# consensus-nexus/bayesian-consensus-engine

Measured on AMD Instinct MI355X. Metric: signals aggregated/sec (node) at 1M markets×32 signals; % of HBM roofline, higher is better.
Workload: dtype f64; 1 GPU; c2: 1000000 markets x 32 signals, 10000 sources, batched consensus + validation + sourceWeights outputs, mode=exact; markets_per_gpu=1000000, signals_per_market=32, parallelism=markets sharded, 1 independent rank(s), no collective

## Files before the change

### bayesian-consensus-engine_amd/csrc/consensus_tab.hip

```cpp
#include <stdio.h>
#include <stdlib.h>

#include <algorithm>

#include "consensus_common.hpp"

#pragma clang fp contract(off)

namespace bce {
namespace {

constexpr int kTabWaves = 8;
constexpr bool kTabMetaEarly = true;
constexpr int kPL = 8;
constexpr int kLB = 3;
constexpr int kMG = 64 / kPL;
constexpr int kTabRing = 8;

typedef unsigned tab_u4v __attribute__((ext_vector_type(4)));
typedef double tab_d2v __attribute__((ext_vector_type(2)));
__device__ __forceinline__ uint4 tab_ld16(const uint32_t* p) {
  const tab_u4v v = __builtin_nontemporal_load(reinterpret_cast<const tab_u4v*>(p));
  return make_uint4(v.x, v.y, v.z, v.w);
}
__device__ __forceinline__ void tab_st16(int32_t* p, uint4 v) {
  const tab_u4v x = {v.x, v.y, v.z, v.w};
  __builtin_nontemporal_store(x, reinterpret_cast<tab_u4v*>(p));
}
__device__ __forceinline__ void tab_st16(double* p, double x0, double x1) {
  const tab_d2v x = {x0, x1};
  __builtin_nontemporal_store(x, reinterpret_cast<tab_d2v*>(p));
}

__device__ __forceinline__ void bfly_pl32(uint32_t& a, uint32_t& b) {
  const auto r = __builtin_amdgcn_permlane32_swap(a, b, false, false);
  a = r[0];
  b = r[1];
}
__device__ __forceinline__ void bfly_pl16(uint32_t& a, uint32_t& b) {
  const auto r = __builtin_amdgcn_permlane16_swap(a, b, false, false);
  a = r[0];
  b = r[1];
}
__device__ __forceinline__ void bfly_r8(uint32_t& a, uint32_t& b, int lane) {
  const bool hi = (lane & 8) != 0;
  const uint32_t bx = (uint32_t)__builtin_amdgcn_mov_dpp((int)b, 0x128, 0xF, 0xF, true);
  const uint32_t ax = (uint32_t)__builtin_amdgcn_mov_dpp((int)a, 0x128, 0xF, 0xF, true);
  const uint32_t na = hi ? bx : a;
  b = hi ? b : ax;
  a = na;
}
template <int N>
__device__ __forceinline__ void xpose(uint32_t (&r)[N], int lane) {
#pragma unroll
  for (int i = 0; i < N; ++i)
    if (!(i & 16)) bfly_pl32(r[i], r[i | 16]);
#pragma unroll
  for (int i = 0; i < N; ++i)
    if (!(i & 8)) bfly_pl16(r[i], r[i | 8]);
#pragma unroll
  for (int i = 0; i < N; ++i)
    if (!(i & 4)) bfly_r8(r[i], r[i | 4], lane);
}

__device__ __forceinline__ int tmkt(int lane) { return lane; }
__device__ __forceinline__ int lq(int lane) { return lane & 7; }
__device__ __forceinline__ int lc(int lane) { return lane >> 3; }
__device__ __forceinline__ void oem_sort_kv31(unsigned (&key)[32], double (&val)[32]) {
  constexpr auto P = OemNet<32>::make();
#pragma unroll
  for (int c = 0; c < OemNet<32>::C; ++c) {
    const unsigned x = key[P.a[c]], y = key[P.b[c]];
    unsigned m = (unsigned)((int)(y - x) >> 31);
    asm("" : "+v"(m));
    key[P.a[c]] = min(x, y);
    key[P.b[c]] = max(x, y);
    const uint64_t vx = (uint64_t)__double_as_longlong(val[P.a[c]]), vy = (uint64_t)__double_as_longlong(val[P.b[c]]);
    const uint64_t mm = ((uint64_t)m << 32) | m;
    val[P.a[c]] = __longlong_as_double((long long)((mm & vy) | (~mm & vx)));
    val[P.b[c]] = __longlong_as_double((long long)((mm & vx) | (~mm & vy)));
  }
}

__device__ __forceinline__ double dbl(uint32_t lo, uint32_t hi) {
  return __hiloint2double((int)hi, (int)lo);
}
__device__ __forceinline__ uint32_t lo32(double x) { return (uint32_t)__double_as_longlong(x); }
__device__ __forceinline__ uint32_t hi32(double x) { return (uint32_t)((uint64_t)__double_as_longlong(x) >> 32); }

template <bool HYB>
__global__ __launch_bounds__(64 * kTabWaves) void consensus_tab32_kernel(ConsArgs a) {
  extern __shared__ __attribute__((aligned(16))) unsigned char tab_smem[];
  const int S = a.n_sources > 0 ? a.n_sources : 1;
  const int nwords = (S + 31) >> 5;
  const int rows = HYB ? a.tab_rows : S;
  double2* const sT = reinterpret_cast<double2*>(tab_smem);
  uint32_t* const sB = reinterpret_cast<uint32_t*>(tab_smem + 16 * (size_t)rows);
  if (a.n_sources > 0) {
    int i = threadIdx.x;
    for (; i + 3 * 64 * kTabWaves < rows; i += 4 * 64 * kTabWaves) {
      double2 v[4];
#pragma unroll
      for (int q = 0; q < 4; ++q) v[q] = a.relconf[i + q * 64 * kTabWaves];
#pragma unroll
      for (int q = 0; q < 4; ++q) sT[i + q * 64 * kTabWaves] = v[q];
    }
    for (; i < rows; i += 64 * kTabWaves) sT[i] = a.relconf[i];
    for (int j = threadIdx.x; j < nwords; j += 64 * kTabWaves) sB[j] = a.pbits[j];
  } else if (threadIdx.x == 0) {
    sT[0] = make_double2(0.5, 0.25);
    sB[0] = 0u;
  }
  __syncthreads();

  const int w = __builtin_amdgcn_readfirstlane((int)(threadIdx.x >> 6));
  const unsigned smax = (unsigned)(S - 1);
  const int64_t M = a.n_list;
  const int64_t n_tiles = (M + 63) >> 6;
  const int64_t stride = (int64_t)gridDim.x * kTabWaves;
  const bool do_u = a.usid != nullptr, do_w = a.weight != nullptr, do_nw = a.nweight != nullptr;
  const bool do_any = do_u || do_w || do_nw;

  struct Meta {
    int64_t off;
    int n;
    int64_t B;
    bool reg;
  };
  auto meta = [&](int64_t tile, int lane) -> Meta {
    Meta m{0, 0, 0, false};
    if (tile >= n_tiles) return m;
    const int j = tmkt(lane);
    const int64_t mk = tile * 64 + j;
    int64_t end = 0;
    if (mk < M) {
      m.off = a.offsets[mk];
      end = a.offsets[mk + 1];
    }
    m.n = (int)(end - m.off);
    if (ballot(mk < M && (m.n < 0 || m.n > 32))) {
      raise_fault(a.fault, kFaultTooLong);
      if (m.n < 0 || m.n > 32) m.n = 0;
    }
    m.B = ((int64_t)__builtin_amdgcn_readfirstlane((int)(m.off >> 32)) << 32) |
          (uint32_t)__builtin_amdgcn_readfirstlane((int)m.off);
    m.reg = ballot(!(mk < M && m.n == 32 && m.off == m.B + 32 * (int64_t)j)) == 0 &&
            ((((uintptr_t)(a.sid + m.B)) | ((uintptr_t)(a.prob + m.B))) & 15) == 0;
    return m;
  };
  auto load_regular = [&](int64_t B, int lane, uint32_t (&rs)[32], uint32_t (&rp)[64]) {
    const int q = lq(lane), c = lc(lane);
    const uint32_t* sb = reinterpret_cast<const uint32_t*>(a.sid + B);
    const double* pb = a.prob + B;
#pragma unroll
    for (int k = 0; k < 8; ++k) {
      const uint4 v = tab_ld16(sb + 32 * (kMG * (k & (kPL - 1)) + q) + 4 * kPL * (k >> kLB) + 4 * c);
      rs[4 * k] = v.x; rs[4 * k + 1] = v.y; rs[4 * k + 2] = v.z; rs[4 * k + 3] = v.w;
    }
#pragma unroll
    for (int k = 0; k < 16; ++k) {
      const uint4 v = tab_ld16(reinterpret_cast<const uint32_t*>(pb + 32 * (kMG * (k & (kPL - 1)) + q) +
                                                                 2 * kPL * (k >> kLB) + 2 * c));
      rp[4 * k] = v.x; rp[4 * k + 1] = v.y; rp[4 * k + 2] = v.z; rp[4 * k + 3] = v.w;
    }
  };

  int64_t tile = (int64_t)w * gridDim.x + blockIdx.x;
  Meta cur = meta(tile, lane_id());
  uint32_t s[32], pw[64];
  for (; tile < n_tiles; tile += stride) {
    int lane = lane_id();
    asm volatile("" : "+v"(lane));
    const int64_t m0 = tile * 64;
    const int64_t off = cur.off, B = cur.B;
    const int n = cur.n;
    const bool reg = cur.reg;
    Meta nxt{};
    if constexpr (kTabMetaEarly) nxt = meta(tile + stride, lane);

    if (reg) {
      load_regular(B, lane, s, pw);
      xpose<32>(s, lane);
      xpose<64>(pw, lane);
    } else if (a.n_signals > 0) {
      const int64_t base = (n > 0) ? off : 0;
      const int last = (n > 0) ? n - 1 : 0;
#pragma unroll
      for (int t = 0; t < 32; ++t) {
        const int64_t i = base + min(t, last);
        s[t] = (uint32_t)a.sid[i];
        const double v = a.prob[i];
        pw[2 * t] = lo32(v);
        pw[2 * t + 1] = hi32(v);
      }
    } else {
#pragma unroll
      for (int t = 0; t < 64; ++t) pw[t] = 0u;
#pragma unroll
      for (int t = 0; t < 32; ++t) s[t] = 0u;
    }
    __builtin_amdgcn_sched_barrier(0);
    double p[32];
#pragma unroll
    for (int t = 0; t < 32; ++t) p[t] = dbl(pw[2 * t], pw[2 * t + 1]);

    const unsigned vb = (n >= 32) ? 0xFFFFFFFFu : ((1u << n) - 1u);
    unsigned badp = 0, bads = 0;
#pragma unroll
    for (int t = 0; t < 32; ++t) {
      badp |= ((p[t] < 0.0 || p[t] > 1.0) ? 1u : 0u) << t;
      bads |= ((s[t] > smax) ? 1u : 0u) << t;
    }
    badp &= vb;
    const int err = badp ? (int)__builtin_ctz(badp) : -1;
    if (ballot((bads & vb) != 0u)) raise_fault(a.fault, kFaultSid);

    unsigned key[32];
#pragma unroll
    for (int t = 0; t < 32; ++t) {
      const uint32_t m = (uint32_t)__builtin_amdgcn_sbfe(vb, t, 1);
      key[t] = (m & ((min(s[t], smax) << 5) | (unsigned)t)) | (~m & 0x7FFFFFFFu);
    }
    oem_sort_kv31(key, p);
    __builtin_amdgcn_sched_barrier(0);
    unsigned nq = 0;
#pragma unroll
    for (int t = 30; t >= 0; --t) nq = (nq << 1) | ((((key[t] ^ key[t + 1]) >> 5) != 0u) ? 1u : 0u);
    const unsigned lb = (nq | 0x80000000u) & vb;
    const unsigned fb = ((nq << 1) | 1u) & vb;

    unsigned dupend = lb & ~fb;
    while (ballot(dupend != 0u)) {
      const int te = dupend ? 31 - __builtin_clz(dupend) : -1;
      const unsigned upto = (te >= 0) ? (0xFFFFFFFFu >> (31 - te)) : 0u;
      dupend &= ~(upto ^ (upto >> 1));
      const unsigned fm = fb & upto;
      const int ts = fm ? 31 - __builtin_clz(fm) : 0;
      const unsigned run = upto & ~((1u << ts) - 1u);
      double psum = 0.0;
#pragma unroll
      for (int t = 0; t < 32; ++t) {
        uint32_t m = (uint32_t)__builtin_amdgcn_sbfe(run, t, 1);
        asm("" : "+v"(m));
        const uint64_t m64 = ((uint64_t)m << 32) | m;
        psum += __longlong_as_double((long long)(m64 & (uint64_t)__double_as_longlong(p[t])));
      }
      const double avg = psum / (double)(te - ts + 1);
      const unsigned at = upto ^ (upto >> 1);
#pragma unroll
      for (int t = 0; t < 32; ++t) {
        uint32_t m = (uint32_t)__builtin_amdgcn_sbfe(at, t, 1);
        asm("" : "+v"(m));
        const uint64_t m64 = ((uint64_t)m << 32) | m;
        p[t] = __longlong_as_double((long long)((m64 & (uint64_t)__double_as_longlong(avg)) |
                                                (~m64 & (uint64_t)__double_as_longlong(p[t]))));
      }
    }
    __builtin_amdgcn_sched_barrier(0);

    __builtin_amdgcn_s_setprio(1);
    double2 ring[kTabRing];
    uint32_t rbits[kTabRing];
    auto row = [&](unsigned ix) -> double2 {
      if constexpr (HYB) {
        if (ix >= (unsigned)rows) return a.relconf[ix];
      }
      return sT[ix];
    };
#pragma unroll
    for (int t = 0; t < kTabRing; ++t) {
      const unsigned ix = min(key[t] >> 5, smax);
      ring[t] = row(ix);
      rbits[t] = sB[ix >> 5];
    }
    double total = 0.0, ws = 0.0, cs = 0.0;
#pragma unroll
    for (int t = 0; t < 32; ++t) {
      const unsigned sid = key[t] >> 5;
      const double2 rc = ring[t % kTabRing];
      const uint32_t bw = rbits[t % kTabRing];
      if (t + kTabRing < 32) {
        const unsigned ix = min(key[t + kTabRing < 32 ? t + kTabRing : t] >> 5, smax);
        ring[t % kTabRing] = row(ix);
        rbits[t % kTabRing] = sB[ix >> 5];
      }
      const double wt = rc.x, cf = rc.y, avg = p[t];
      const bool lst = ((lb >> t) & 1u) != 0u;
      total += lst ? wt : 0.0;
      ws += lst ? avg * wt : 0.0;
      cs += lst ? cf * wt : 0.0;
      key[t] = sid | ((((bw >> (sid & 31)) & 1u) != 0u) ? 0u : 0x80000000u);
      p[t] = wt;
      asm volatile("" : "+v"(total), "+v"(ws), "+v"(cs));
      __builtin_amdgcn_sched_barrier(0);
    }
    const int u = __builtin_popcount(lb);

    __builtin_amdgcn_s_setprio(2);
    if constexpr (!kTabMetaEarly) nxt = meta(tile + stride, lane_id());
    {
      int ln = lane_id();
      asm volatile("" : "+v"(ln));
      const int64_t mk2 = m0 + tmkt(ln);
      if (mk2 < M) {
        const bool null_ = (total == 0.0);
        a.consensus[mk2] = null_ ? 0.0 : ws / total;
        a.confidence[mk2] = null_ ? 0.0 : cs / total;
        a.total_weight[mk2] = total;
        a.n_unique[mk2] = u;
        if (a.err_idx) a.err_idx[mk2] = err;
      }
    }
    if (!do_any) {
      __builtin_amdgcn_s_setprio(0);
      cur = nxt;
      continue;
    }

    const unsigned full = (u >= 32) ? 0xFFFFFFFFu : ((1u << u) - 1u);
    if (ballot(lb != full)) {
      unsigned holes = vb & ~lb;
      while (ballot(holes != 0u)) {
        const int h = holes ? 31 - __builtin_clz(holes) : 32;
        holes &= ~(1u << (h & 31));
#pragma unroll
        for (int i = 0; i < 31; ++i) {
          uint32_t m = (uint32_t)((h - 1 - i) >> 31);
          asm("" : "+v"(m));
          key[i] = (m & key[i + 1]) | (~m & key[i]);
          const uint64_t m64 = ((uint64_t)m << 32) | m;
          const uint64_t x = (uint64_t)__double_as_longlong(p[i + 1]), y = (uint64_t)__double_as_longlong(p[i]);
          p[i] = __longlong_as_double((long long)((m64 & x) | (~m64 & y)));
        }
      }
    }

    __builtin_amdgcn_s_setprio(3);
    __builtin_amdgcn_sched_barrier(0);
    if (reg) {
      uint32_t blo = (uint32_t)B, bhi = (uint32_t)((uint64_t)B >> 32);
      asm volatile("" : "+s"(blo), "+s"(bhi));
      const int64_t B = (int64_t)(((uint64_t)bhi << 32) | blo);
      int lane = lane_id();
      asm volatile("" : "+v"(lane));
      const int q = lq(lane), c = lc(lane);
      int uk[kPL];
      double tk[kPL];
#pragma unroll
      for (int k = 0; k < kPL; ++k) {
        const int src = ((k << 3) | (lane & 7)) << 2;
        uk[k] = __builtin_amdgcn_ds_bpermute(src, u);
        tk[k] = dbl((uint32_t)__builtin_amdgcn_ds_bpermute(src, (int)lo32(total)),
                    (uint32_t)__builtin_amdgcn_ds_bpermute(src, (int)hi32(total)));
      }
      if (do_u) {
        uint32_t o[32];
#pragma unroll
        for (int t = 0; t < 32; ++t) o[t] = key[t];
        xpose<32>(o, lane);
#pragma unroll
        for (int k = 0; k < 8; ++k) {
          const int slot = 4 * kPL * (k >> kLB) + 4 * c;
          if (uk[k & (kPL - 1)] > slot)
            tab_st16(a.usid + B + 32 * (kMG * (k & (kPL - 1)) + q) + slot,
                     make_uint4(o[4 * k], o[4 * k + 1], o[4 * k + 2], o[4 * k + 3]));
        }
      }
      if (do_w || do_nw) {
        uint32_t o[64];
#pragma unroll
        for (int t = 0; t < 32; ++t) {
          o[2 * t] = lo32(p[t]);
          o[2 * t + 1] = hi32(p[t]);
        }
        xpose<64>(o, lane);
#pragma unroll
        for (int k = 0; k < 16; ++k) {
          const int slot = 2 * kPL * (k >> kLB) + 2 * c;
          const int64_t pos = B + 32 * (kMG * (k & (kPL - 1)) + q) + slot;
          const double w0 = dbl(o[4 * k], o[4 * k + 1]), w1 = dbl(o[4 * k + 2], o[4 * k + 3]);
          const double tot = tk[k & (kPL - 1)];
          if (uk[k & (kPL - 1)] > slot) {
            if (do_w) tab_st16(a.weight + pos, w0, w1);
            if (do_nw) tab_st16(a.nweight + pos, tot > 0.0 ? w0 / tot : 0.0, tot > 0.0 ? w1 / tot : 0.0);
          }
        }
      }
    } else {
      int ln = lane_id();
      asm volatile("" : "+v"(ln));
      const int64_t mk2 = m0 + tmkt(ln);
      const int64_t off = (mk2 < M) ? a.offsets[mk2] : 0;
#pragma unroll
      for (int j = 0; j < 32; ++j) {
        if (j < u) {
          if (do_u) a.usid[off + j] = (int32_t)key[j];
          if (do_w) a.weight[off + j] = p[j];
        }
      }
      if (do_nw) {
#pragma unroll
        for (int j = 0; j < 32; ++j) {
          const double v = total > 0.0 ? p[j] / total : 0.0;
          if (j < u) a.nweight[off + j] = v;
        }
      }
    }
    __builtin_amdgcn_s_setprio(0);
    cur = nxt;
  }
}

}


template <bool HYB>
int launch_tab32_t(ConsArgs a, hipStream_t st) {
  const int64_t tiles = (a.n_list + 63) / 64;
  if (tiles == 0) return BCE_OK;
  const int S = a.n_sources > 0 ? a.n_sources : 1;
  const size_t bits = 4 * (size_t)((S + 31) / 32);
  a.tab_rows = HYB ? (int)std::min<size_t>(((size_t)kTabLdsBytes - bits) / 16, (size_t)S) : S;
  const size_t lds = 16 * (size_t)a.tab_rows + bits;
  const void* fn = reinterpret_cast<const void*>(&consensus_tab32_kernel<HYB>);
  const int rc = ensure_dynamic_lds(fn, kTabLdsBytes);
  if (rc) return rc;
  const int per_cu = blocks_per_cu(fn, 64 * kTabWaves, lds, 1, HYB ? "consensus_tab32_kernel<hybrid>"
                                                                  : "consensus_tab32_kernel");
  const int64_t blocks = (tiles + kTabWaves - 1) / kTabWaves;
  const int64_t cap = (int64_t)cu_count() * per_cu;
  const int grid = (int)(blocks < cap ? blocks : cap);
  hipLaunchKernelGGL((consensus_tab32_kernel<HYB>), dim3(grid), dim3(64 * kTabWaves), lds, st, a);
  return check_launch("consensus_tab32_kernel");
}

int launch_tab32(const ConsArgs& a, hipStream_t st) {
  return (a.n_sources <= kTabMaxSources) ? launch_tab32_t<false>(a, st) : launch_tab32_t<true>(a, st);
}

}
```

Measured before the change: 149.3 billion signals/s.

## Specialize tile body for regular tiles and overlap offsets prefetch with loads

Splits the per-tile loop body into a compile-time specialized lambda for regular (full 32-signal, contiguous) tiles and an irregular fallback. This drops the validity-mask work in key construction for the common case. Offset metadata is now issued as raw loads and finished later. The first tile's offsets load overlaps the LDS table fill, and the next tile's offsets load is issued after the bulk signal loads so it sits behind them. Metadata is kept in scalar registers, but duplicating the body roughly doubles code size and may raise instruction-cache and register pressure.

New measurement: 151.1 billion signals/s, median of 3. About the same (+1.2%).

```diff
diff --git a/bayesian-consensus-engine_amd/csrc/consensus_tab.hip b/bayesian-consensus-engine_amd/csrc/consensus_tab.hip
--- a/bayesian-consensus-engine_amd/csrc/consensus_tab.hip
+++ b/bayesian-consensus-engine_amd/csrc/consensus_tab.hip
@@ -2,6 +2,7 @@
 #include <stdlib.h>
 
 #include <algorithm>
+#include <type_traits>
 
 #include "consensus_common.hpp"
 
@@ -11,7 +12,6 @@
 namespace {
 
 constexpr int kTabWaves = 8;
-constexpr bool kTabMetaEarly = true;
 constexpr int kPL = 8;
 constexpr int kLB = 3;
 constexpr int kMG = 64 / kPL;
@@ -82,6 +82,12 @@
   }
 }
 
+__device__ __forceinline__ int lane_here() {
+  unsigned ones = ~0u;
+  asm volatile("" : "+s"(ones));
+  return (int)__builtin_amdgcn_mbcnt_hi(ones, __builtin_amdgcn_mbcnt_lo(ones, 0u));
+}
+
 __device__ __forceinline__ double dbl(uint32_t lo, uint32_t hi) {
   return __hiloint2double((int)hi, (int)lo);
 }
@@ -96,6 +102,18 @@
   const int rows = HYB ? a.tab_rows : S;
   double2* const sT = reinterpret_cast<double2*>(tab_smem);
   uint32_t* const sB = reinterpret_cast<uint32_t*>(tab_smem + 16 * (size_t)rows);
+  const int w = __builtin_amdgcn_readfirstlane((int)(threadIdx.x >> 6));
+  const int64_t M = a.n_list;
+  const int64_t n_tiles = (M + 63) >> 6;
+  int64_t tile = (int64_t)w * gridDim.x + blockIdx.x;
+  struct RawMeta {
+    int64_t off, end;
+  };
+  auto meta_issue = [&](int64_t t, int lane) -> RawMeta {
+    const int64_t mk = min(t * 64 + tmkt(lane), M - 1);
+    return RawMeta{a.offsets[mk], a.offsets[mk + 1]};
+  };
+  const RawMeta raw0 = meta_issue(tile, lane_id());
   if (a.n_sources > 0) {
     int i = threadIdx.x;
     for (; i + 3 * 64 * kTabWaves < rows; i += 4 * 64 * kTabWaves) {
@@ -113,40 +131,30 @@
   }
   __syncthreads();
 
-  const int w = __builtin_amdgcn_readfirstlane((int)(threadIdx.x >> 6));
   const unsigned smax = (unsigned)(S - 1);
-  const int64_t M = a.n_list;
-  const int64_t n_tiles = (M + 63) >> 6;
   const int64_t stride = (int64_t)gridDim.x * kTabWaves;
   const bool do_u = a.usid != nullptr, do_w = a.weight != nullptr, do_nw = a.nweight != nullptr;
   const bool do_any = do_u || do_w || do_nw;
 
-  struct Meta {
-    int64_t off;
-    int n;
+  struct Head {
     int64_t B;
     bool reg;
   };
-  auto meta = [&](int64_t tile, int lane) -> Meta {
-    Meta m{0, 0, 0, false};
-    if (tile >= n_tiles) return m;
+  auto meta_finish = [&](const RawMeta& r, int64_t t, int lane) -> Head {
     const int j = tmkt(lane);
-    const int64_t mk = tile * 64 + j;
-    int64_t end = 0;
-    if (mk < M) {
-      m.off = a.offsets[mk];
-      end = a.offsets[mk + 1];
-    }
-    m.n = (int)(end - m.off);
-    if (ballot(mk < M && (m.n < 0 || m.n > 32))) {
-      raise_fault(a.fault, kFaultTooLong);
-      if (m.n < 0 || m.n > 32) m.n = 0;
-    }
-    m.B = ((int64_t)__builtin_amdgcn_readfirstlane((int)(m.off >> 32)) << 32) |
-          (uint32_t)__builtin_amdgcn_readfirstlane((int)m.off);
-    m.reg = ballot(!(mk < M && m.n == 32 && m.off == m.B + 32 * (int64_t)j)) == 0 &&
-            ((((uintptr_t)(a.sid + m.B)) | ((uintptr_t)(a.prob + m.B))) & 15) == 0;
-    return m;
+    const bool in = t * 64 + j < M;
+    const int n = (int)(r.end - r.off);
+    if (ballot(in && (n < 0 || n > 32))) raise_fault(a.fault, kFaultTooLong);
+    uint32_t blo = (uint32_t)__builtin_amdgcn_readfirstlane((int)r.off);
+    uint32_t bhi = (uint32_t)__builtin_amdgcn_readfirstlane((int)(r.off >> 32));
+    const int64_t B0 = (int64_t)(((uint64_t)bhi << 32) | blo);
+    uint32_t reg = (uint32_t)__builtin_amdgcn_readfirstlane(
+        (ballot(!(in && n == 32 && r.off == B0 + 32 * (int64_t)j)) == 0 &&
+         ((((uintptr_t)(a.sid + B0)) | ((uintptr_t)(a.prob + B0))) & 15) == 0)
+            ? 1
+            : 0);
+    asm volatile("" : "+s"(blo), "+s"(bhi), "+s"(reg));
+    return Head{(int64_t)(((uint64_t)bhi << 32) | blo), reg != 0u};
   };
   auto load_regular = [&](int64_t B, int lane, uint32_t (&rs)[32], uint32_t (&rp)[64]) {
     const int q = lq(lane), c = lc(lane);
@@ -165,46 +173,52 @@
     }
   };
 
-  int64_t tile = (int64_t)w * gridDim.x + blockIdx.x;
-  Meta cur = meta(tile, lane_id());
+  Head cur = meta_finish(raw0, tile, lane_id());
   uint32_t s[32], pw[64];
-  for (; tile < n_tiles; tile += stride) {
-    int lane = lane_id();
-    asm volatile("" : "+v"(lane));
+  auto tile_body = [&](auto R, const int64_t B) __attribute__((always_inline)) -> Head {
+    constexpr bool REG = decltype(R)::value;
+    const int lane = lane_here();
     const int64_t m0 = tile * 64;
-    const int64_t off = cur.off, B = cur.B;
-    const int n = cur.n;
-    const bool reg = cur.reg;
-    Meta nxt{};
-    if constexpr (kTabMetaEarly) nxt = meta(tile + stride, lane);
-
-    if (reg) {
+    int n = 32;
+    RawMeta raw;
+
+    if constexpr (REG) {
       load_regular(B, lane, s, pw);
+      raw = meta_issue(tile + stride, lane);
       xpose<32>(s, lane);
       xpose<64>(pw, lane);
-    } else if (a.n_signals > 0) {
-      const int64_t base = (n > 0) ? off : 0;
-      const int last = (n > 0) ? n - 1 : 0;
-#pragma unroll
-      for (int t = 0; t < 32; ++t) {
-        const int64_t i = base + min(t, last);
-        s[t] = (uint32_t)a.sid[i];
-        const double v = a.prob[i];
-        pw[2 * t] = lo32(v);
-        pw[2 * t + 1] = hi32(v);
-      }
+      __builtin_amdgcn_sched_barrier(0);
+      asm volatile("" : "+v"(raw.off), "+v"(raw.end), "+v"(pw[63]), "+v"(s[31]));
     } else {
-#pragma unroll
-      for (int t = 0; t < 64; ++t) pw[t] = 0u;
-#pragma unroll
-      for (int t = 0; t < 32; ++t) s[t] = 0u;
-    }
+      const RawMeta me = meta_issue(tile, lane);
+      n = (int)(me.end - me.off);
+      if (!(m0 + tmkt(lane) < M) || n < 0 || n > 32) n = 0;
+      if (a.n_signals > 0) {
+        const int64_t base = (n > 0) ? me.off : 0;
+        const int last = (n > 0) ? n - 1 : 0;
+#pragma unroll
+        for (int t = 0; t < 32; ++t) {
+          const int64_t i = base + min(t, last);
+          s[t] = (uint32_t)a.sid[i];
+          const double v = a.prob[i];
+          pw[2 * t] = lo32(v);
+          pw[2 * t + 1] = hi32(v);
+        }
+      } else {
+#pragma unroll
+        for (int t = 0; t < 64; ++t) pw[t] = 0u;
+#pragma unroll
+        for (int t = 0; t < 32; ++t) s[t] = 0u;
+      }
+      raw = meta_issue(tile + stride, lane);
+    }
+    const Head nxt = meta_finish(raw, tile + stride, lane);
     __builtin_amdgcn_sched_barrier(0);
     double p[32];
 #pragma unroll
     for (int t = 0; t < 32; ++t) p[t] = dbl(pw[2 * t], pw[2 * t + 1]);
 
-    const unsigned vb = (n >= 32) ? 0xFFFFFFFFu : ((1u << n) - 1u);
+    const unsigned vb = (REG || n >= 32) ? 0xFFFFFFFFu : ((1u << n) - 1u);
     unsigned badp = 0, bads = 0;
 #pragma unroll
     for (int t = 0; t < 32; ++t) {
@@ -218,8 +232,12 @@
     unsigned key[32];
 #pragma unroll
     for (int t = 0; t < 32; ++t) {
-      const uint32_t m = (uint32_t)__builtin_amdgcn_sbfe(vb, t, 1);
-      key[t] = (m & ((min(s[t], smax) << 5) | (unsigned)t)) | (~m & 0x7FFFFFFFu);
+      if constexpr (REG) {
+        key[t] = (min(s[t], smax) << 5) | (unsigned)t;
+      } else {
+        const uint32_t m = (uint32_t)__builtin_amdgcn_sbfe(vb, t, 1);
+        key[t] = (m & ((min(s[t], smax) << 5) | (unsigned)t)) | (~m & 0x7FFFFFFFu);
+      }
     }
     oem_sort_kv31(key, p);
     __builtin_amdgcn_sched_barrier(0);
@@ -291,16 +309,14 @@
       cs += lst ? cf * wt : 0.0;
       key[t] = sid | ((((bw >> (sid & 31)) & 1u) != 0u) ? 0u : 0x80000000u);
       p[t] = wt;
-      asm volatile("" : "+v"(total), "+v"(ws), "+v"(cs));
+      asm volatile("" : "+v"(total), "+v"(ws), "+v"(cs), "+v"(key[t]));
       __builtin_amdgcn_sched_barrier(0);
     }
     const int u = __builtin_popcount(lb);
 
     __builtin_amdgcn_s_setprio(2);
-    if constexpr (!kTabMetaEarly) nxt = meta(tile + stride, lane_id());
     {
-      int ln = lane_id();
-      asm volatile("" : "+v"(ln));
+      const int ln = lane_here();
       const int64_t mk2 = m0 + tmkt(ln);
       if (mk2 < M) {
         const bool null_ = (total == 0.0);
@@ -313,8 +329,7 @@
     }
     if (!do_any) {
       __builtin_amdgcn_s_setprio(0);
-      cur = nxt;
-      continue;
+      return nxt;
     }
 
     const unsigned full = (u >= 32) ? 0xFFFFFFFFu : ((1u << u) - 1u);
@@ -337,12 +352,11 @@
 
     __builtin_amdgcn_s_setprio(3);
     __builtin_amdgcn_sched_barrier(0);
-    if (reg) {
+    if constexpr (REG) {
       uint32_t blo = (uint32_t)B, bhi = (uint32_t)((uint64_t)B >> 32);
       asm volatile("" : "+s"(blo), "+s"(bhi));
       const int64_t B = (int64_t)(((uint64_t)bhi << 32) | blo);
-      int lane = lane_id();
-      asm volatile("" : "+v"(lane));
+      const int lane = lane_here();
       const int q = lq(lane), c = lc(lane);
       int uk[kPL];
       double tk[kPL];
@@ -387,8 +401,7 @@
         }
       }
     } else {
-      int ln = lane_id();
-      asm volatile("" : "+v"(ln));
+      const int ln = lane_here();
       const int64_t mk2 = m0 + tmkt(ln);
       const int64_t off = (mk2 < M) ? a.offsets[mk2] : 0;
 #pragma unroll
@@ -407,8 +420,10 @@
       }
     }
     __builtin_amdgcn_s_setprio(0);
-    cur = nxt;
-  }
+    return nxt;
+  };
+  for (; tile < n_tiles; tile += stride)
+    cur = cur.reg ? tile_body(std::true_type{}, cur.B) : tile_body(std::false_type{}, cur.B);
 }
 
 }
```
